# medical-genomics-group/hydra

Hardware: AMD Instinct MI355X
Metric: Gibbs markers/sec/iter (higher is better)
Workload: dtype f64

## Files before the change

### hydra_amd/capi.py

```python
import ctypes as C
import os
import numpy as np

_HERE = os.path.dirname(os.path.abspath(__file__))
LIB_PATH = os.path.join(_HERE, "libhgibbs.so")

ABI_SYMBOLS = [
    "hgibbs_last_error", "hgibbs_version", "hgibbs_create", "hgibbs_destroy", "hgibbs_comm_unique_id",
    "hgibbs_comm_init", "hgibbs_comm_init_external", "hgibbs_p2p_export", "hgibbs_p2p_import", "hgibbs_load_bed", "hgibbs_synth_bed", "hgibbs_dims", "hgibbs_get_bed",
    "hgibbs_marker_stats", "hgibbs_set_residual", "hgibbs_get_residual", "hgibbs_reduce_eps", "hgibbs_add_scalar",
    "hgibbs_update_marker", "hgibbs_dot_marker", "hgibbs_set_covariates", "hgibbs_cov_dot", "hgibbs_cov_update",
    "hydra_chain_set_covariates", "hydra_chain_gamma", "hgibbs_set_components", "hydra_chain_restore",
    "hydra_rng_to_boost_words", "hydra_rng_from_boost_words", "hydra_rng_shuffle", "hgibbs_set_model", "hgibbs_set_beta", "hgibbs_get_beta",
    "hgibbs_beta_sqnorm", "hgibbs_sweep", "hgibbs_set_option", "hgibbs_last_sweep_stats", "hgibbs_stream_ceiling", "hgibbs_debug_times", "hgibbs_resident_trace", "hydra_chain_create",
    "hydra_chain_destroy", "hydra_chain_iterate", "hydra_chain_state", "hydra_chain_csv_line", "hydra_chain_order",
    "hydra_chain_last_nnz", "hgibbs_score", "hgibbs_last_score_ms", "hgibbs_ld", "hgibbs_last_ld_ms",
    "hgibbs_ld_scores", "hgibbs_last_ld_scores_ms",
    "hgibbs_ld_mask", "hgibbs_last_ld_mask_ms", "hgibbs_ld_greedy", "hgibbs_ld_clump",
    "hgibbs_marker_dots", "hgibbs_last_marker_dots_ms", "hgibbs_marker_class_sums", "hgibbs_last_marker_class_sums_ms", "hgibbs_logit_null",
    "hgibbs_spa_roots", "hgibbs_last_spa_ms", "hgibbs_spa_pvalue",
    "hgibbs_king", "hgibbs_king_pairs", "hgibbs_king_pairs_get", "hgibbs_last_king_ms",
    "hgibbs_pca", "hgibbs_last_pca_ms", "hgibbs_region_var", "hgibbs_last_region_var_ms",
    "hgibbs_grm", "hgibbs_grm_info", "hgibbs_last_grm_ms",
    "hgibbs_grm_rowsums", "hgibbs_last_grm_rowsums_ms", "hgibbs_he_fit",
    "hgibbs_row_sums", "hgibbs_last_row_sums_ms", "hgibbs_hwe_exact",
    "hgibbs_sparse_begin", "hgibbs_sparse_put", "hgibbs_sparse_end", "hgibbs_sparse_counts", "hgibbs_sparse_get", "hgibbs_last_sparse_ms",
    "hgibbs_grand_seed", "hgibbs_grand_next", "hgibbs_ars_sample", "hgibbs_w_init", "hgibbs_w_marker_stats", "hgibbs_w_set_model",
    "hgibbs_w_reduce", "hgibbs_w_refresh_vi", "hgibbs_w_get_vi", "hgibbs_w_marker_sums", "hgibbs_w_sweep", "hgibbs_w_last_sweep_stats", "hgibbs_w_ars_device_probe",
    "hgibbs_w_get_beta", "hgibbs_w_set_beta", "hydraw_chain_create", "hydraw_chain_destroy", "hydraw_chain_set_covariates",
    "hydraw_chain_reseed_ars", "hydraw_chain_iterate", "hydraw_chain_state", "hydraw_chain_gamma", "hydraw_chain_order",
    "hydraw_chain_last_nnz", "hydraw_chain_csv_line", "hydraw_chain_restore",
]


class RngState(C.Structure):
    _fields_ = [("x", C.c_uint32 * 624), ("idx", C.c_uint32)]


class SweepStats(C.Structure):
    _fields_ = [("launches", C.c_uint64), ("nnz_updates", C.c_uint64), ("device_ms", C.c_double),
                ("kernel_ms_avg", C.c_double), ("carried_columns", C.c_uint64), ("working_launches", C.c_uint64),
                ("accepted_markers", C.c_uint64), ("streamed_columns", C.c_uint64), ("tiles_per_workgroup_min", C.c_uint32),
                ("tiles_per_workgroup_max", C.c_uint32), ("engine", C.c_uint32), ("walker", C.c_uint32), ("eps_sum_drift", C.c_double),
                ("rounds", C.c_uint64), ("events", C.c_uint64), ("advances", C.c_uint64), ("chunks", C.c_uint64), ("refolds", C.c_uint64), ("pivots", C.c_uint64), ("predicted", C.c_uint64), ("shader_mhz", C.c_double),
                ("ticks", C.c_uint64 * 16), ("refill", C.c_uint32), ("reserved_", C.c_uint32)]


class PcaReport(C.Structure):
    _fields_ = [("iters_run", C.c_int32), ("m_used", C.c_uint32), ("ritz_change", C.c_double), ("resid", C.c_double * 32)]


class SpaRoot(C.Structure):
    _fields_ = [("t", C.c_double * 2), ("K", C.c_double * 2), ("K2", C.c_double * 2), ("k2_0", C.c_double), ("s_lo", C.c_double),
                ("s_hi", C.c_double), ("iters", C.c_int32 * 2), ("flags", C.c_uint32), ("reserved_", C.c_uint32)]


class HeForm(C.Structure):
    _fields_ = [(k, C.c_double) for k in ("intercept", "slope", "h2", "intercept_se", "slope_se", "h2_se", "intercept_se_jk", "slope_se_jk",
                                         "h2_se_jk", "intercept_p", "slope_p", "intercept_p_jk", "slope_p_jk")]

# ... 91 lines not shown
    L.hgibbs_cov_dot.argtypes = [vp, C.c_int, C.c_double, dp]
    L.hgibbs_cov_update.argtypes = [vp, C.c_int, C.c_double]
    L.hydra_chain_set_covariates.argtypes = [vp, dp, C.c_int]
    L.hydra_chain_gamma.argtypes = [vp, dp, ip]
    L.hgibbs_set_components.argtypes = [vp, ip]
    L.hydra_chain_restore.argtypes = [vp, C.POINTER(RestartState)]
    L.hydra_rng_to_boost_words.argtypes = [C.POINTER(RngState), u32p]
    L.hydra_rng_from_boost_words.argtypes = [u32p, C.POINTER(RngState)]
    L.hydra_rng_shuffle.argtypes = [C.POINTER(RngState), ip, C.c_uint32]
    L.hgibbs_set_model.argtypes = [vp, C.c_int, C.c_int, ip, dp, dp]
    L.hgibbs_set_beta.argtypes = [vp, dp]
    L.hgibbs_get_beta.argtypes = [vp, dp, ip, dp]
    L.hgibbs_beta_sqnorm.argtypes = [vp, dp]
    L.hgibbs_sweep.argtypes = [vp, ip, C.c_double, dp, dp, u8p, C.POINTER(RngState), ip, u64p]
    L.hgibbs_set_option.argtypes = [vp, C.c_char_p, C.c_int64]
    L.hgibbs_last_sweep_stats.argtypes = [vp, C.POINTER(SweepStats)]
    L.hgibbs_stream_ceiling.argtypes = [vp, C.c_uint64, C.c_int, dp]
    L.hgibbs_debug_times.argtypes = [vp, C.POINTER(C.c_uint64)]
    L.hgibbs_resident_trace.argtypes = [vp, C.POINTER(C.c_uint64), C.c_uint64]
    L.hydra_chain_create.argtypes = [vp, C.POINTER(ModelDesc), dp, C.POINTER(vp)]
    L.hydra_chain_destroy.argtypes = [vp]
    L.hydra_chain_iterate.argtypes = [vp]
    L.hydra_chain_state.argtypes = [vp, dp, dp, dp, dp, ip, ip, C.POINTER(RngState)]
    L.hydra_chain_csv_line.argtypes = [vp, C.c_uint32, C.c_char_p, C.c_size_t]
    L.hydra_chain_order.argtypes = [vp]
    L.hydra_chain_order.restype = ip
    L.hydra_chain_last_nnz.argtypes = [vp]
    gp = C.POINTER(GrandState)
    L.hgibbs_grand_seed.argtypes = [gp, C.c_uint32]
    L.hgibbs_grand_seed.restype = None
# ... 636 lines not shown
        return cass, nnz.value

    def resident_trace(self):
        out = np.zeros((10, 4096), dtype=np.uint64)
        check(self.L.hgibbs_resident_trace(self.h, out.ctypes.data_as(C.POINTER(C.c_uint64)), out.size))
        return out

    def sweep_stats(self):
        s = SweepStats()
        check(self.L.hgibbs_last_sweep_stats(self.h, C.byref(s)))
        return {"launches": s.launches, "nnz_updates": s.nnz_updates, "device_ms": s.device_ms,
                "kernel_ms_avg": s.kernel_ms_avg, "carried_columns": s.carried_columns, "working_launches": s.working_launches,
                "accepted_markers": s.accepted_markers, "streamed_columns": s.streamed_columns,
                "tiles_per_workgroup_min": s.tiles_per_workgroup_min, "tiles_per_workgroup_max": s.tiles_per_workgroup_max,
                "engine": s.engine, "walker": s.walker, "refill": s.refill, "eps_sum_drift": s.eps_sum_drift, "rounds": s.rounds, "events": s.events,
                "advances": s.advances, "chunks": s.chunks, "refolds": s.refolds, "pivots": s.pivots, "predicted": s.predicted, "shader_mhz": s.shader_mhz, "ticks": list(s.ticks)}


class Chain:

    def __init__(self, dev, y, mS=None, groups=None, seed=1222, shuffle=1):
        self.dev = dev
        self.L = dev.L
        if mS is None:
            mS = np.array([[0.0, 0.0001, 0.001, 0.01]])
        self.mS = np.ascontiguousarray(mS, dtype=np.float64)
        self.G, self.K = self.mS.shape
        self.groups = None if groups is None else np.ascontiguousarray(groups, dtype=np.int32)
        y = np.ascontiguousarray(y, dtype=np.float64)
        assert y.shape[0] == dev.n_global
        d = ModelDesc(seed, shuffle, self.G, self.K, _ip(self.groups) if self.groups is not None else None, _dp(self.mS))
# ... 222 lines not shown
```

### hydra_amd/csrc/hg_resident.hip.h

```cpp
#pragma once

#include "hg_sweep.hip.h"

namespace hg {

constexpr int RS_WAVES = 8;
constexpr int RS_BLOCK = RS_WAVES * WAVE;
constexpr int RS_BMAX = 256;
constexpr int RS_NSH = 8;
constexpr int RS_RSH = 8;
constexpr int RS_GROW = 1024;
constexpr int RS_CROW = 1024;
constexpr int RS_RB = 2 * RS_BMAX;
constexpr int RS_MSG = 16;
constexpr int RS_PMAX = 4;
constexpr int RS_PFIRE = 16;
constexpr int RS_NB = 256;
constexpr int RS_TRACE = 4096;
constexpr int RS_TMAX = 2;
constexpr uint32_t RS_ONE = 1u << 24;
constexpr uint32_t RS_LOW = RS_ONE - 1u;
constexpr unsigned long long RS_ONE64 = 1ull << 56;
constexpr int RS_GFX = 32;
constexpr int RS_FG = 4, RS_FN = 256;
// ... 11 lines not shown
    uint32_t x = seq * 0x9E3779B1u ^ lo ^ (hi * 0x85EBCA77u);
    x ^= x >> 16;
    return x & 0xffffu;
}
constexpr unsigned long long RS_RONE = 1ull << 56;
__host__ __device__ inline unsigned long long rs_raw_value(unsigned long long d) { return (unsigned long long)((long long)(d << 8) >> 8); }
__host__ __device__ inline uint32_t rs_raw_count(unsigned long long d) { return (uint32_t)((d - rs_raw_value(d)) >> 56) & 0xffu; }
__host__ __device__ inline uint32_t rs_window_end(uint32_t C, uint32_t B, uint32_t M, uint32_t mask)
{
    const uint32_t e = (C + B) & ~mask;
    return e < M ? e : M;
}
__host__ __device__ inline uint32_t rs_msg_word0(uint32_t kf, uint32_t ncons, uint32_t seq, uint32_t lo, uint32_t hi) { return (kf << 28) | (rs_msg_check(seq, lo, hi) << 12) | ncons; }

struct ResState {
    uint32_t cursor, rng_idx, error, pad;
    unsigned long long rounds, events, advances, nnz, chunks, refolds, pivots, predicted;
    unsigned long long shader_ticks, wall_ticks;
    unsigned long long t[16];
};

struct ResParams {
    const uint8_t* bed;
    uint64_t stride;
    double* eps;
    uint32_t n_pad, n_local, M;
    double n_minus_1, n_total, eps_sum;
    const int32_t* order;
    const double* s_mave;
    const double* s_mstd;
    const double* s_bold;
// ... 18 lines not shown
    unsigned long long* racc;
    uint32_t* rcnt;
    unsigned long long* racc2;
    unsigned long long* gacc64;
    const unsigned long long* counts;
    unsigned long long* pacc;
    ResMsg* msg;
    ResState* state;
    double fx_scale, fx_unscale;
    unsigned long long timeout;
    unsigned long long* progress;
    unsigned long long rdv_timeout;
    unsigned long long* trace;
    int dbg;
    int pivots;
    int unused_;
    int early_advance;
    uint32_t wend_mask;
    int announce;
    int walker;
    const uint32_t* pred;
    int all_ada;
    int nranks, rank;
    unsigned char* mbox[RX_MAXR];
    unsigned long long sweep_id;
};

constexpr uint32_t RX_RING = 1024;
constexpr size_t RX_GBOX = 0;
constexpr size_t RX_RBOX = RX_GBOX + (size_t)RX_MAXR * 2 * RS_BMAX * 16;
constexpr size_t RX_HBOX = RX_RBOX + (size_t)RX_MAXR * RX_RING * 32;
// ... 1865 lines not shown
```

### hydra_amd/csrc/hg_walker2.hip.h

```cpp
#pragma once

namespace hg {

constexpr int W2_NBLK = 4;
constexpr uint32_t W2_RING = W2_NBLK * MT_N;
constexpr uint32_t W2_RR = 1024;
constexpr uint32_t W2_EV = 64;
constexpr uint32_t W2_PRED = 1024;
constexpr uint32_t W2_NB = 256;
constexpr int W2_NCH = 4;
constexpr uint32_t W2_NREC = 8;

enum {
    S_FPUB = 0,
    S_MPUB,
    S_CPUB,
    S_SEQPUB,
    S_RECSEQ,
    S_BLK,
    S_GPOS,
    S_PLD,
    S_PCUR,
    S_RDONE,
    S_EVN,
// ... 13 lines not shown
    R_FD,
    R_SEQ,
    R_PIN,
    R_PIQ,
    R_NEV,
    R_GPOSR,
    R_PFN,
    R_DB = 12,
    R_MQ = 14,
    R_SQ = 16,
    R_GSQ = 18,
    R_NMQ = 20,
    R_WORDS = 32
};
enum { RT_EXTEND = 0, RT_ADVANCE = 1, RT_PIVOT = 2, RT_EVENT = 3, RT_END = 4 };
enum { W2_ST_ROUNDS = 0, W2_ST_EVENTS, W2_ST_ADV, W2_ST_NNZ, W2_ST_CHUNKS, W2_ST_REFOLD, W2_ST_PIVOTS, W2_ST_PRED, W2_ST_ANN };

#define W2_ARRAYS(X)                                                                                                                          \
    X(double, tq, (size_t)W2_RING)         \
    X(double, zig_nx, 130)                                                                                                                    \
    X(double, zig_ny, 130)                                                                                                                    \
    X(double, htab, (size_t)4 * HT_LDS)                                                                                                       \
    X(double, qtab, (size_t)2 * HT_LDS)                                                                                                       \
    X(double, ftab, (size_t)RS_FG * (RS_FN + 1))                                                                                              \
    X(double, fscale, RS_FG)                                                                                                                  \
    X(double, mave, MR)                                                                               \
    X(double, mstd, MR)                                                                                                                       \
    X(double, bold, MR)                                                                                                                       \
    X(double, gsum, MR)                                                                                                     \
    X(double, nmis, MR)                                                                                                                       \
    X(double, dpr, Bz)                                                                               \
// ... 89 lines not shown
__device__ __forceinline__ Walk2Lds walk2_lds(uint32_t B)
{
    Walk2Lds sh;
    const Walk2Off off = walk2_offsets(B);
    uint32_t lb = (uint32_t)__builtin_amdgcn_readfirstlane((int)(uint32_t)(uintptr_t)(W2_LDS unsigned char*)hg_smem);
    asm volatile("" : "+s"(lb));
    W2_LDS unsigned char* const lbase = (W2_LDS unsigned char*)(uintptr_t)lb;
#define W2_X(type, name, count) sh.name = (W2_LDS type*)(lbase + off.name);
    W2_ARRAYS(W2_X)
#undef W2_X
    return sh;
}

#define W2_BEXPR pr.B
#define W2_PIVEXPR (pr.pivots != 0)
#define W2_PROLOGUE \
    const int tid = threadIdx.x, lane = tid & 63; \
    const int wave = __builtin_amdgcn_readfirstlane(tid >> 6); \
    const uint32_t B = W2_BEXPR, bmask = B - 1u, M = pr.M; \
    const uint32_t MR = 2u * B, mrmask = MR - 1u; \
    const int K = pr.K, GK = pr.GK; \
    const uint32_t W = pr.W, nsh = pr.nsh, rsh = pr.rsh; \
    const double n_total = pr.n_total, n_minus_1 = pr.n_minus_1, i_2sigE = pr.i_2sigE, eps_sum = pr.eps_sum, fx_unscale = pr.fx_unscale; \
    const unsigned long long timeout = pr.timeout; \
    const bool pivots = W2_PIVEXPR; \
    const uint32_t early_advance = (uint32_t)pr.early_advance; \
    const bool announce = pr.announce != 0 && !pivots; \
    const uint32_t rng_idx0 = pr.rng_idx; \
    ResMsg* const msg = pr.msg; \
    ResState* const state = pr.state; \
    unsigned long long* const trace = pr.trace; \
    unsigned long long* const progress = pr.progress; \
    const uint32_t* const gpred = pr.pred; \
    const double* const zig_ex = pr.zig.ex; \
    const double* const zig_ey = pr.zig.ey; \
    const Walk2Lds sh = walk2_lds(B); \
// ... 9 lines not shown
        const int ga = pr.s_ga[j]; \
        const int mk = pr.order[j]; \
        sh.marker[ms] = mk; \
        sh.ga[ms] = ga; \
        sh.bold[ms] = pr.s_bold[j]; \
        sh.mave[ms] = pr.s_mave[j]; \
        sh.mstd[ms] = pr.s_mstd[j]; \
        if constexpr (MISS) { \
            const unsigned long long* cn = pr.counts + 3ull * (unsigned long long)mk; \
            sh.gsum[ms] = (double)(cn[0] + 2ull * cn[1]); \
            sh.nmis[ms] = (double)cn[2]; \
        } \
    }; \
    auto tq_of = [&](uint32_t word) { \
        const double prob = (double)mt_temper(word) * (1.0 / 4294967296.0); \
        return log(1.0 / prob - 1.0) - 1e-9; \
    }; \
    auto aborted = [&]() { return w2_ld(sh.sw + S_ABORT) != 0u; }; \
    auto ended = [&]() { return w2_ld(sh.sw + S_END) != 0u; };

template <int DBG, int MISS, int BC, int RANKS, int DECIDE, int PIV>
__device__ __attribute__((noinline)) void w2_chain(const ResParams& prg)
{
    typedef const __attribute__((address_space(4))) ResParams w2_cparams;
    const unsigned long long pga = (unsigned long long)(uintptr_t)&prg;
    const unsigned long long pgu = ((unsigned long long)(uint32_t)__builtin_amdgcn_readfirstlane((int)(uint32_t)(pga >> 32)) << 32) |
                                   (uint32_t)__builtin_amdgcn_readfirstlane((int)(uint32_t)pga);
    w2_cparams& pr = *(w2_cparams*)(uintptr_t)pgu;
#undef W2_BEXPR
#define W2_BEXPR (BC ? (uint32_t)BC : pr.B)
#undef W2_PIVEXPR
#define W2_PIVEXPR (PIV != 0)
    W2_PROLOGUE
#undef W2_BEXPR
#define W2_BEXPR pr.B
#undef W2_PIVEXPR
#define W2_PIVEXPR (pr.pivots != 0)
    __builtin_amdgcn_s_setprio(3);
    constexpr bool decider = DECIDE != 0;
    const uint32_t nch = B >= 64u ? B / 64u : 1u;
    const uint32_t slot = (uint32_t)wave * 64u + (uint32_t)lane;
    const bool son = slot < B;
    const uint32_t sl = son ? slot : 0u;
    double dpr = 0.0, dp = 0.0, mave = 0.0, mstd = 0.0, boldn = 0.0, fsc = 0.0, gsm = 0.0, nms = 0.0;
    uint32_t fof = 0, sbt = 0, spi = 0;
    bool prd = false;
    uint32_t C = 0, Sx = 0, Fs = 0, base = 0, gposr = rng_idx0 % W2_RING;
    uint32_t gpa32[RS_NSH], gpb32[RS_NSH];
    unsigned long long gpa64[RS_NSH], gpb64[RS_NSH];
#pragma unroll
    for (int r = 0; r < RS_NSH; ++r) {
        gpa32[r] = gpb32[r] = 0u;
        gpa64[r] = gpb64[r] = 0ull;
    }
    typedef const __attribute__((address_space(1))) uint32_t* w2_g32;
    typedef const __attribute__((address_space(1))) unsigned long long* w2_g64;
    const w2_g32 gacc = (w2_g32)pr.gacc;
    const w2_g64 gacc64 = (w2_g64)pr.gacc64;
    uint32_t rno = 0;

    uint32_t seq = 0, nev = 0, pi = 0, evn = 0, pf_n = 0, gpos = rng_idx0, blk = 1u;
    uint32_t rdone_seen = 0, wpub_seen = 0, evw_seen = 0, pld_seen = W2_PRED, fpub_seen = 0, mpub_seen = m0;
    unsigned long long cm[W2_NCH] = {0ull, 0ull, 0ull, 0ull};
    uint32_t stat = 0;
    auto count = [&](uint32_t bits) { stat += (bits >> (uint32_t)lane) & 1u; };
    uint32_t err = 0;
    bool failed = false;
    unsigned long long tacc[8] = {0ull, 0ull, 0ull, 0ull, 0ull, 0ull, 0ull, 0ull};
    unsigned long long tmark = DBG ? wall_clock64() : 0ull;
    auto lap = [&](int i) {
        if (DBG && decider) {
            const unsigned long long now = wall_clock64();
            tacc[i] += now - tmark;
            tmark = now;
        }
    };
    auto pos_of_slot = [&](uint32_t s, uint32_t c) { return c + ((s - c) & bmask); };
    uint32_t nspin = 0;
// ... 263 lines not shown
            const int kx = inside ? (int)x : 0;
            uint32_t r = gposr + ((j - C) & bmask);
            r = r >= W2_RING ? r - W2_RING : r;
            const double f0 = sh.ftab[fof + (uint32_t)kx], f1 = sh.ftab[fof + (uint32_t)kx + 1u], tqv = sh.tq[r];
            const double fup = f0 + (x - (double)kx) * (f1 - f0);
            mymask = __ballot(act && (prd || !(inside && fup <= tqv)));
        }
        base = Fs;
        if (!decider) {
            if (lane == 0) *(W2_LDS u4_t*)(sh.ans + 4 * wave) = rs_u4((uint32_t)mymask, (uint32_t)(mymask >> 32), rno + 1u, 0u);
            ++rno;
            continue;
        }
        ++rno;
        lap(5);
        if (r_type != (uint32_t)RT_EXTEND) cm[0] = cm[1] = cm[2] = cm[3] = 0ull;
        cm[0] |= mymask;
        if (nch > 1u) {
            const unsigned long long t0 = wall_clock64();
            for (;;) {
                const u4_t a1 = *(const volatile W2_LDS u4_t*)(sh.ans + 4), a2 = *(const volatile W2_LDS u4_t*)(sh.ans + 8), a3 = *(const volatile W2_LDS u4_t*)(sh.ans + 12);
                const bool ok = w2_uni(a1.z) == rno && (nch < 3u || (w2_uni(a2.z) == rno && w2_uni(a3.z) == rno));
                if (ok) {
                    cm[1] |= ((unsigned long long)w2_uni(a1.y) << 32) | w2_uni(a1.x);
                    if (nch >= 3u) {
                        cm[2] |= ((unsigned long long)w2_uni(a2.y) << 32) | w2_uni(a2.x);
                        cm[3] |= ((unsigned long long)w2_uni(a3.y) << 32) | w2_uni(a3.x);
                    }
                    break;
                }
                if (spin_fail(t0)) {
                    failed = true;
                    break;
                }
            }
        }
        if (failed) break;
        lap(1);
        const uint32_t fc_rdone = __hip_atomic_load(sh.sw + S_RDONE, __ATOMIC_RELAXED, __HIP_MEMORY_SCOPE_WORKGROUP),
                       fc_wpub = __hip_atomic_load(sh.sw + S_WPUB, __ATOMIC_RELAXED, __HIP_MEMORY_SCOPE_WORKGROUP),
                       fc_evw = __hip_atomic_load(sh.sw + S_EVW, __ATOMIC_RELAXED, __HIP_MEMORY_SCOPE_WORKGROUP);
        if (lane == W2_ST_CHUNKS && (DBG || (stat & 255u) == 0u)) w2_gst(progress, ((unsigned long long)(uint32_t)__builtin_amdgcn_readlane((int)stat, W2_ST_ROUNDS) << 8) | 1u);
        if (PIV && pf_n) {
            if (Fs >= Sx) pf_n = 0;
            else {
                const uint32_t bF = w2_uni(sh.batch[Fs & bmask]);
                uint32_t drop = 0;
                while (drop < pf_n && w2_uni(sh.pf_msg[drop]) <= bF) ++drop;
                if (drop) {
                    if (lane == 0)
                        for (uint32_t f = drop; f < pf_n; ++f) {
                            sh.pf_pos[f - drop] = sh.pf_pos[f];
// ... 3 lines not shown
                            sh.pf_val[3 * (f - drop) + 1] = sh.pf_val[3 * f + 1];
                            sh.pf_val[3 * (f - drop) + 2] = sh.pf_val[3 * f + 2];
                        }
                    pf_n -= drop;
                    w2_lds_done();
                }
            }
        }
        if (gpos + B + 96u > blk * (uint32_t)MT_N && !wait_seen(blk, S_BLK, (gpos + B + 96u + (uint32_t)MT_N - 1u) / (uint32_t)MT_N)) break;
        count(1u << W2_ST_CHUNKS);
        bool found = false, announced = false;
        uint32_t qpos = 0, q_consumed = 0;
        int q_k = 0;
        double q_bnew = 0.0, q_bold = 0.0, q_mq = 0.0, q_sq = 0.0, q_gsq = 0.0, q_nmq = 0.0;
        {
            const uint32_t s0 = C & bmask, i0 = s0 >> 6, l0 = s0 & 63u;
            const unsigned long long lowm = (1ull << l0) - 1ull;
            for (;;) {
                uint32_t qs = 0xffffffffu;
#pragma unroll
                for (int t = 0; t <= W2_NCH; ++t) {
                    if ((uint32_t)t <= nch && qs == 0xffffffffu) {
                        uint32_t i = i0 + (uint32_t)t;
                        i = i >= nch ? i - nch : i;
                        unsigned long long mm = i == 0u ? cm[0] : (i == 1u ? cm[1] : (i == 2u ? cm[2] : cm[3]));
                        if (t == 0) mm &= ~lowm;
                        if ((uint32_t)t == nch) mm &= lowm;
                        if (mm) qs = i * 64u + (uint32_t)(__ffsll((long long)mm) - 1);
                    }
                }
                qs = w2_uni(qs);
                if (qs == 0xffffffffu) break;
                const uint32_t qc = pos_of_slot(qs, C);
                const uint32_t qi = qs >> 6, ql = qs & 63u;
                const uint32_t ms = qc & mrmask;
                uint32_t upos = gposr + (qc - C);
                upos = upos >= W2_RING ? upos - W2_RING : upos;
                const double bold_v = sh.bold[ms], num = sh.rnum[qc & (W2_RR - 1u)];
                const double cmq_v = sh.mave[ms], csq_v = sh.mstd[ms], cgsq_v = MISS ? sh.gsum[ms] : 0.0, cnmq_v = MISS ? sh.nmis[ms] : 0.0;
                const int ga_v = sh.ga[ms];
                const uint32_t word_v = sh.mt[upos];
                const uint32_t zp1 = upos + 1u == W2_RING ? 0u : upos + 1u, zp2 = zp1 + 1u == W2_RING ? 0u : zp1 + 1u;
                const uint32_t zw1 = sh.mt[zp1], zw2 = sh.mt[zp2];
                const double bold = w2_uni(bold_v);
                if (announce && !announced && bold != 0.0 && qc + 1u < Sx && (seq + 6u <= (uint32_t)RS_MSG || rdone_seen >= seq + 6u - (uint32_t)RS_MSG)) {
                    if (lane == 0) rs_store16(msg + ((seq + 1u) % RS_MSG), rs_u4(rs_msg_word0((uint32_t)RS_ANNOUNCE, qc - C + 1u, seq + 1u, 0u, 0u), seq + 1u, 0u, 0u));
                    announced = true;
                }
                const uint32_t zleft = blk * (uint32_t)MT_N - (gpos + (qc - C) + 1u);
// ... 18 lines not shown
                    const int lk = lane < K ? lane : 0;
                    const double den = sh.htab[g0 + lk], lpi = sh.htab[HT_LDS + g0 + lk], hlg = sh.htab[2 * HT_LDS + g0 + lk];
                    sdl = sh.htab[3 * HT_LDS + g0 + lk];
                    mk = num / (lk ? den : 1.0);
                    Lm = lk ? lpi - hlg + mk * num * i_2sigE : lpi;
                }
                const int kk = lane >> 3, l = lane & 7;
                const double Ll = __shfl(Lm, l, 64), Lk = __shfl(Lm, kk, 64);
                const bool on = kk < K - 1 && l < K;
                const double d = on ? Ll - Lk : 0.0;
                const double ex = exp(d);
                const bool bigp = on && l >= (kk ? kk : 1) && fabs(d) > 700.0;
                const unsigned long long bm = __ballot(bigp);
                double sum = ex, cur = ex;
#pragma unroll
                for (int x = 1; x < 8; ++x) {
                    cur = rs_dpp_f64<0x101>(cur);
                    if (x < K) sum += cur;
                }
                const bool anyb = ((bm >> (lane & ~7)) & 0xffull) != 0ull;
                const double thr = anyb ? 0.0 : 1.0 / sum;
                int k = K - 1;
                double acum = 0.0;
                bool fnd = false;
#pragma unroll
                for (int sidx = 0; sidx < 7; ++sidx) {
                    if (sidx + 1 < K) {
                        const double t = rs_readlane(thr, 8 * sidx);
                        acum = sidx ? acum + t : t;
                        if (!fnd && prob <= acum) {
                            k = sidx;
                            fnd = true;
                        }
                    }
                }
                k = w2_uni(k);
                double bnew = 0.0;
                uint32_t consumed = 0u, gerr = 0u;
                if (k > 0) {
                    const double mean_k = rs_readlane(mk, k), sd_k = rs_readlane(sdl, k);
                    if (zfast) {
                        bnew = z * sd_k + mean_k;
                        consumed = 2u;
                    } else {
                        if (lane == 0) {
                            RingGen g{sh.mt, zp1, zleft, 0u, 0u};
                            const ZigLds zt{sh.zig_nx, sh.zig_ny, zig_ex, zig_ey};
// ... 12 lines not shown
                    break;
                }
                if (k != 0 || bold != 0.0) {
                    found = true;
                    q_mq = w2_uni(cmq_v);
                    q_sq = w2_uni(csq_v);
                    q_gsq = w2_uni(cgsq_v);
                    q_nmq = w2_uni(cnmq_v);
                    qpos = qc;
                    q_k = k;
                    q_bnew = bnew;
                    q_bold = bold;
                    q_consumed = consumed;
                    break;
                }
                const unsigned long long bit = 1ull << ql;
                if (qi == 0u) cm[0] &= ~bit;
                else if (qi == 1u) cm[1] &= ~bit;
                else if (qi == 2u) cm[2] &= ~bit;
                else cm[3] &= ~bit;
            }
        }
        lap(3);
        if (failed) break;
        const uint32_t early_thr = early_advance;
        const bool early = !found && Fs < Sx && early_thr != 0u && Fs - C >= early_thr;
        if (!found && Fs < Sx && !early) {
            count(1u << W2_ST_REFOLD);
            if (!wait_seen(fpub_seen, S_FPUB, Fs + 1u)) break;
            lap(0);
            publish(RT_EXTEND, 0u, C, Sx, Sx, fpub_seen < Sx ? fpub_seen : Sx, 0u, 0.0, 0.0, 0.0, 0.0, 0.0);
            continue;
        }
        const uint32_t ncons = found ? qpos - C + 1u : (early ? Fs - C : Sx - C);
        const uint32_t Cn = C + ncons;
// ... 95 lines not shown
        publish(RT_END, 0u, C, Sx, Sx, 0u, 0u, 0.0, 0.0, 0.0, 0.0, 0.0);
        if (lane == 0) {
            w2_st(sh.sw + S_GPOS, gpos);
            w2_lds_done();
            w2_st(sh.sw + S_END, 1u);
            state->cursor = C;
            auto st = [&](int i) { return (uint32_t)__builtin_amdgcn_readlane((int)stat, i); };
            state->rounds = st(W2_ST_ROUNDS);
            state->events = st(W2_ST_EVENTS);
            state->advances = st(W2_ST_ADV);
            state->nnz = st(W2_ST_NNZ);
            state->chunks = st(W2_ST_CHUNKS);
            state->refolds = st(W2_ST_REFOLD);
            state->pivots = st(W2_ST_PIVOTS) + st(W2_ST_ANN);
            state->predicted = st(W2_ST_PRED);
            if (DBG)
                for (int i = 0; i < 8; ++i) state->t[i] = tacc[i];
        }
    }
}

template <int MISS, int RANKS>
__device__ __attribute__((noinline)) void w2_folder(const ResParams& pr)
{
    W2_PROLOGUE
    uint32_t Ff = 0, done = 0, fb = 0;
    unsigned long long t_idle = wall_clock64();
    auto poll_done = [&]() {
        uint32_t b = 0xffffffffu;
        if ((uint32_t)lane < rsh) b = __hip_atomic_load(pr.rcnt + (size_t)lane * RS_CROW, HG_RLX_AGENT) / cntR[(uint32_t)lane < W % rsh ? 0 : 1];
#pragma unroll
        for (int off = 32; off >= 1; off >>= 1) {
            const uint32_t o = (uint32_t)__shfl_xor((int)b, off, 64);
            b = o < b ? o : b;
// ... 329 lines not shown
        uint32_t np = 0;
        for (int ip = 0; ip < RS_PMAX; ++ip) np += (pivots && sh.pred[ip] < Sx0) ? 1u : 0u;
        sh.bl_pi[0] = 0u;
        sh.bl_np[0] = np;
        sh.bl_p0[0] = np ? sh.pred[0] : 0xffffffffu;
    }
    __syncthreads();

    if (wave < W2_NCH) {
        if ((uint32_t)wave < (B >= 64u ? B / 64u : 1u)) {
            if (wave == 0) {
                if (pr.nranks > 1) w2_chain<DBG, MISS, 0, 1, 1, 0>(pr);
                else if (!MISS && pr.pivots) {
                    if (B == 256u) w2_chain<DBG, MISS, 256, 0, 1, 1>(pr);
                    else w2_chain<DBG, MISS, 0, 0, 1, 1>(pr);
                } else if (B == 256u) w2_chain<DBG, MISS, 256, 0, 1, 0>(pr);
                else w2_chain<DBG, MISS, 0, 0, 1, 0>(pr);
            } else {
                if (pr.nranks > 1) w2_chain<DBG, MISS, 0, 1, 0, 0>(pr);
                else if (!MISS && pr.pivots) {
                    if (B == 256u) w2_chain<DBG, MISS, 256, 0, 0, 1>(pr);
                    else w2_chain<DBG, MISS, 0, 0, 0, 1>(pr);
                } else if (B == 256u) w2_chain<DBG, MISS, 256, 0, 0, 0>(pr);
                else w2_chain<DBG, MISS, 0, 0, 0, 0>(pr);
            }
        }
    } else if (wave == 4) {
        if (pr.nranks > 1) w2_folder<MISS, 1>(pr);
        else w2_folder<MISS, 0>(pr);
    }
    else if (wave == 5) w2_housekeeper<MISS>(pr);
    __syncthreads();
// ... 21 lines not shown
```

### hydra_amd/csrc/hgibbs.hip

```cpp
#include <hip/hip_runtime.h>
#include <rccl/rccl.h>

#include <algorithm>
#include <atomic>
#include <chrono>
#include <thread>
#include <cmath>
#include <cstdarg>
#include <cstdio>
#include <cstdlib>
#include <cstring>
#include <string>
#include <vector>

#include "../../include/hgibbs.h"
#include "hg_kernels.h"
#include "hg_sweep.hip.h"
#include "hg_resident.hip.h"

using namespace hg;

static thread_local std::string g_err;

static int fail(const char* fmt, ...)
// ... 117 lines not shown

    int engine = 0;
    bool res_all_ada = false;
    unsigned long long res_sweep_id = 0;
    bool engine_pinned = false;
    uint32_t window = 0;
    uint32_t res_cus = 0;
    int res_walker = 0;
    bool res_attr_set[20] = {};
    bool res_dead = false;
    uint32_t res_probed_w = 0;
    unsigned long long res_probe_id = 0;
    bool res_not_resident = false;
    int res_early = 24;
    int res_announce = 1;
    int res_wend = 1;
    int res_walker2_ranks = 1;
    double eps_abs_bound = 0.0;
    int res_refill = 0;
    int res_pivots = 0;
    unsigned char* res_acc = nullptr;
    ResMsg* res_msg = nullptr;
    ResState* res_state = nullptr;
    ResState* res_state_host = nullptr;
    ResParams* res_params = nullptr;
    ResParams* res_params_host = nullptr;
    unsigned long long* res_progress = nullptr;
    unsigned long long* res_progress_host = nullptr;
    hipStream_t aux_stream = nullptr;
    unsigned long long* res_trace = nullptr;
// ... 1121 lines not shown
        h->window = (uint32_t)value;
    } else if (!std::strcmp(name, "pivots")) {
        h->res_pivots = value != 0;
    } else if (!std::strcmp(name, "early_advance")) {
        if (value < 0 || value > 255) return fail("early_advance must be in [0,255]");
        h->res_early = (int)value;
    } else if (!std::strcmp(name, "refill")) {
        if (value < 0 || value > 2) return fail("refill must be 0 (auto), 1 (fused multiply-adds) or 2 (integer matrix products)");
        h->res_refill = (int)value;
    } else if (!std::strcmp(name, "walker2_ranks")) {
        h->res_walker2_ranks = value != 0;
    } else if (!std::strcmp(name, "window_end16")) {
        h->res_wend = value != 0;
    } else if (!std::strcmp(name, "announce")) {
        h->res_announce = value != 0;
    } else if (!std::strcmp(name, "walker")) {
        if (value < 0 || value > 2) return fail("walker must be 0 (auto), 1 (first) or 2 (second)");
        h->res_walker = (int)value;
    } else if (!std::strcmp(name, "res_cus")) {
        if (value < 0 || value > 4096) return fail("res_cus must be in [0,4096]");
        h->res_cus = (uint32_t)value;
    } else if (!std::strcmp(name, "res_deadline_ms")) {
        h->res_deadline_s = (double)value * 1e-3;
    } else if (!std::strcmp(name, "res_timeout_ms")) {
        if (value < 1) return fail("res_timeout_ms must be positive");
        h->res_timeout_s = (double)value * 1e-3;
    } else if (!std::strcmp(name, "p2p")) {
        h->p2p_enabled = value != 0;
    } else if (!std::strcmp(name, "force_split")) {
        h->force_split = value != 0;
    } else if (!std::strcmp(name, "w_kernel_timing")) {
        h->w_kernel_timing = value != 0;
    } else if (!std::strcmp(name, "debug_timing")) {
        h->debug_timing = value != 0;
    } else if (!std::strcmp(name, "sparse_piece")) {
        if (value < 0) return fail("sparse_piece must be >= 0 bytes (0 = automatic)");
        h->sparse_piece = (long long)value;
    } else if (!std::strcmp(name, "chunk")) {
        h->chunk = (int)value;
    } else {
        return fail("hgibbs_set_option: unknown option '%s'", name);
    }
    return 0;
}

int hgibbs_debug_times(hgibbs_t h, uint64_t* out8)
{
    if (!h || !out8) return fail("null argument");
    HIP_TRY(hipSetDevice(h->device));
    HIP_TRY(hipMemcpy(out8, h->dbg, 48 * sizeof(unsigned long long), hipMemcpyDeviceToHost));
    HIP_TRY(hipMemset(h->dbg, 0, 48 * sizeof(unsigned long long)));
    return 0;
}

int hgibbs_resident_trace(hgibbs_t h, uint64_t* out, uint64_t words)
{
    if (!h || !out) return fail("null argument");
    HIP_TRY(hipSetDevice(h->device));
// ... 200 lines not shown
        p.fx_scale = std::ldexp(1.0, ex);
        p.fx_unscale = std::ldexp(1.0, -ex);
    }
    p.timeout = (unsigned long long)(h->res_timeout_s * 1e8);
    p.rdv_timeout = (unsigned long long)(std::min(h->res_timeout_s, 0.1) * 1e8);
    p.dbg = h->debug_timing ? 1 : 0;
    p.pivots = pl.pivots;
    p.nranks = h->nranks > 1 ? h->nranks : 1;
    p.rank = h->nranks > 1 ? h->rank : 0;
    for (int r = 0; r < RX_MAXR; ++r) p.mbox[r] = (h->nranks > 1 && r < h->nranks) ? (unsigned char*)h->peer_base[r] + MBOX_RES_OFF : nullptr;
    p.all_ada = h->res_all_ada ? 1 : 0;
    p.walker = pl.walker;
    p.pred = h->pred;
    p.early_advance = p.nranks > 1 ? 0 : h->res_early;
    p.announce = h->res_announce;
    p.wend_mask = pl.wend_mask;
    {
        const uint32_t nchunk = (h->M + PRED_CHUNK - 1) / PRED_CHUNK;
        k_pred_count<<<nchunk, 256, 0, h->stream>>>(h->s_bold, h->M, h->pred_cnt);
        k_pred_scan<<<1, 1024, 0, h->stream>>>(h->pred_cnt, nchunk);
        k_pred_scatter<<<nchunk, 256, 0, h->stream>>>(h->s_bold, h->M, h->pred_cnt, nchunk, h->pred, nullptr);
        HIP_TRY(hipGetLastError());
    }
    p.sweep_id = ++h->res_sweep_id;
    p.trace = h->res_trace;
    p.progress = h->res_progress;
    HIP_TRY(hipMemsetAsync(h->res_progress, 0, 16 * sizeof(unsigned long long), h->stream));

    HIP_TRY(hipMemsetAsync(h->res_acc, 0, RES_ACC_BYTES, h->stream));
    HIP_TRY(hipMemsetAsync(h->res_msg, 0, RS_MSG * sizeof(ResMsg), h->stream));
// ... 90 lines not shown
    s.working_launches = st.rounds;
    s.kernel_ms_avg = st.rounds ? ms / (double)st.rounds : 0.0;
    s.accepted_markers = st.cursor;
    s.streamed_columns = h->M;
    s.tiles_per_workgroup_min = s.tiles_per_workgroup_max = (uint32_t)pl.T;
    s.engine = 2;
    s.walker = (uint32_t)pl.walker;
    s.refill = (uint32_t)pl.refill;
    s.rounds = st.rounds;
    s.events = st.events;
    s.advances = st.advances;
    s.chunks = st.chunks;
    s.refolds = st.refolds;
    s.pivots = st.pivots;
    s.predicted = st.predicted;
    for (int i = 0; i < 16; ++i) s.ticks[i] = st.t[i];
    s.shader_mhz = st.wall_ticks ? 100.0 * (double)st.shader_ticks / (double)st.wall_ticks : 0.0;
    {
        double r1[2];
        if (reduce_eps_all(h, r1)) return 1;
        s.eps_sum_drift = std::fabs(r1[0] - r0[0]);
    }
    if (timing) {
        auto ms = [](auto a, auto b) { return std::chrono::duration<double, std::milli>(b - a).count(); };
        std::fprintf(stderr, "[hgibbs] resident sweep: launch preparation %.3f ms, kernel wait %.3f ms (device %.3f), results + drift %.3f\n", ms(t_0, t_launch), ms(t_launch, t_kernel),
                     (double)s.device_ms, ms(t_kernel, std::chrono::steady_clock::now()));
    }
    return 0;
}

// ... 320 lines not shown
```

### include/hgibbs.h

```cpp
#ifndef HGIBBS_H
#define HGIBBS_H

#include <stddef.h>
#include <stdint.h>

#ifdef __cplusplus
extern "C" {
#endif

typedef struct hgibbs_ctx* hgibbs_t;

typedef struct {
    uint32_t x[624];
    uint32_t idx;
} hgibbs_rng_state;

const char* hgibbs_last_error(void);
int hgibbs_version(void);

int hgibbs_create(int device_id, hgibbs_t* out);
int hgibbs_destroy(hgibbs_t h);

int hgibbs_comm_unique_id(void* id128);
int hgibbs_comm_init(hgibbs_t h, int nranks, int rank, const void* id128);
// ... 39 lines not shown
int hgibbs_cov_update(hgibbs_t h, int c, double dgamma);

int hgibbs_set_model(hgibbs_t h, int G, int K, const int32_t* groups_host, const double* cVa_host,
                     const double* cVaI_host);

int hgibbs_set_beta(hgibbs_t h, const double* beta_host);
int hgibbs_set_components(hgibbs_t h, const int32_t* components_host);
int hgibbs_get_beta(hgibbs_t h, double* beta_host, int32_t* components_host, double* acum_host);
int hgibbs_beta_sqnorm(hgibbs_t h, double* bsq_host );

int hgibbs_sweep(hgibbs_t h, const int32_t* order_host, double sigmaE, const double* sigmaG_host,
                 const double* estPi_host, const uint8_t* adaV_host, hgibbs_rng_state* rng, int32_t* cass_host,
                 uint64_t* nnz_updates);

int hgibbs_set_option(hgibbs_t h, const char* name, int64_t value);
typedef struct {
    uint64_t launches;
    uint64_t nnz_updates;
    double device_ms;
    double kernel_ms_avg;
    uint64_t carried_columns;
    uint64_t working_launches;
    uint64_t accepted_markers;
    uint64_t streamed_columns;
    uint32_t tiles_per_workgroup_min;
    uint32_t tiles_per_workgroup_max;
    uint32_t engine;
    uint32_t walker;
    double eps_sum_drift;
    uint64_t rounds, events, advances, chunks, refolds;
    uint64_t pivots;
    uint64_t predicted;
    double shader_mhz;
    uint64_t ticks[16];
    uint32_t refill;
    uint32_t reserved_;
} hgibbs_sweep_stats;
int hgibbs_last_sweep_stats(hgibbs_t h, hgibbs_sweep_stats* out);
int hgibbs_stream_ceiling(hgibbs_t h, uint64_t bytes, int reps, double* gbps);
int hgibbs_debug_times(hgibbs_t h, uint64_t* out48);
int hgibbs_resident_trace(hgibbs_t h, uint64_t* out, uint64_t words);

int hgibbs_score(hgibbs_t h, int S, const double* a, const double* o, double* out);
int hgibbs_last_score_ms(hgibbs_t h, double* ms);

int hgibbs_row_sums(hgibbs_t h, int T, const double* tab, double* out);
int hgibbs_last_row_sums_ms(hgibbs_t h, double* ms);

int hgibbs_hwe_exact(uint32_t n_het, uint32_t n_hom_a, uint32_t n_hom_b, double* p);

int hgibbs_region_var(hgibbs_t h, int S, const double* a, const double* o, uint32_t nsets, const uint64_t* off, const uint32_t* idx,
// ... 190 lines not shown
```

Baseline: 9.379 million.

## Specialize walker2 chain for K=4 and keep candidate masks in lane registers

```diff
diff --git a/hydra_amd/capi.py b/hydra_amd/capi.py
--- a/hydra_amd/capi.py
+++ b/hydra_amd/capi.py
@@ -12,7 +12,7 @@
     "hgibbs_update_marker", "hgibbs_dot_marker", "hgibbs_set_covariates", "hgibbs_cov_dot", "hgibbs_cov_update",
     "hydra_chain_set_covariates", "hydra_chain_gamma", "hgibbs_set_components", "hydra_chain_restore",
     "hydra_rng_to_boost_words", "hydra_rng_from_boost_words", "hydra_rng_shuffle", "hgibbs_set_model", "hgibbs_set_beta", "hgibbs_get_beta",
-    "hgibbs_beta_sqnorm", "hgibbs_sweep", "hgibbs_set_option", "hgibbs_last_sweep_stats", "hgibbs_stream_ceiling", "hgibbs_debug_times", "hgibbs_resident_trace", "hydra_chain_create",
+    "hgibbs_beta_sqnorm", "hgibbs_sweep", "hgibbs_set_option", "hgibbs_walker_search", "hgibbs_last_sweep_stats", "hgibbs_stream_ceiling", "hgibbs_debug_times", "hgibbs_resident_trace", "hydra_chain_create",
     "hydra_chain_destroy", "hydra_chain_iterate", "hydra_chain_state", "hydra_chain_csv_line", "hydra_chain_order",
     "hydra_chain_last_nnz", "hgibbs_score", "hgibbs_last_score_ms", "hgibbs_ld", "hgibbs_last_ld_ms",
     "hgibbs_ld_scores", "hgibbs_last_ld_scores_ms",
@@ -43,7 +43,7 @@
                 ("accepted_markers", C.c_uint64), ("streamed_columns", C.c_uint64), ("tiles_per_workgroup_min", C.c_uint32),
                 ("tiles_per_workgroup_max", C.c_uint32), ("engine", C.c_uint32), ("walker", C.c_uint32), ("eps_sum_drift", C.c_double),
                 ("rounds", C.c_uint64), ("events", C.c_uint64), ("advances", C.c_uint64), ("chunks", C.c_uint64), ("refolds", C.c_uint64), ("pivots", C.c_uint64), ("predicted", C.c_uint64), ("shader_mhz", C.c_double),
-                ("ticks", C.c_uint64 * 16), ("refill", C.c_uint32), ("reserved_", C.c_uint32)]
+                ("ticks", C.c_uint64 * 16), ("refill", C.c_uint32), ("turned_down", C.c_uint32)]
 
 
 class PcaReport(C.Structure):
@@ -165,6 +165,7 @@
     L.hgibbs_beta_sqnorm.argtypes = [vp, dp]
     L.hgibbs_sweep.argtypes = [vp, ip, C.c_double, dp, dp, u8p, C.POINTER(RngState), ip, u64p]
     L.hgibbs_set_option.argtypes = [vp, C.c_char_p, C.c_int64]
+    L.hgibbs_walker_search.argtypes = [u64p, C.c_uint32, C.c_uint32, u32p, C.c_uint32]
     L.hgibbs_last_sweep_stats.argtypes = [vp, C.POINTER(SweepStats)]
     L.hgibbs_stream_ceiling.argtypes = [vp, C.c_uint64, C.c_int, dp]
     L.hgibbs_debug_times.argtypes = [vp, C.POINTER(C.c_uint64)]
@@ -831,7 +832,7 @@
                 "accepted_markers": s.accepted_markers, "streamed_columns": s.streamed_columns,
                 "tiles_per_workgroup_min": s.tiles_per_workgroup_min, "tiles_per_workgroup_max": s.tiles_per_workgroup_max,
                 "engine": s.engine, "walker": s.walker, "refill": s.refill, "eps_sum_drift": s.eps_sum_drift, "rounds": s.rounds, "events": s.events,
-                "advances": s.advances, "chunks": s.chunks, "refolds": s.refolds, "pivots": s.pivots, "predicted": s.predicted, "shader_mhz": s.shader_mhz, "ticks": list(s.ticks)}
+                "advances": s.advances, "chunks": s.chunks, "refolds": s.refolds, "pivots": s.pivots, "predicted": s.predicted, "turned_down": s.turned_down, "shader_mhz": s.shader_mhz, "ticks": list(s.ticks)}
 
 
 class Chain:
diff --git a/hydra_amd/csrc/hg_resident.hip.h b/hydra_amd/csrc/hg_resident.hip.h
--- a/hydra_amd/csrc/hg_resident.hip.h
+++ b/hydra_amd/csrc/hg_resident.hip.h
@@ -49,7 +49,7 @@
 __host__ __device__ inline uint32_t rs_msg_word0(uint32_t kf, uint32_t ncons, uint32_t seq, uint32_t lo, uint32_t hi) { return (kf << 28) | (rs_msg_check(seq, lo, hi) << 12) | ncons; }
 
 struct ResState {
-    uint32_t cursor, rng_idx, error, pad;
+    uint32_t cursor, rng_idx, error, turned_down;
     unsigned long long rounds, events, advances, nnz, chunks, refolds, pivots, predicted;
     unsigned long long shader_ticks, wall_ticks;
     unsigned long long t[16];
@@ -98,7 +98,7 @@
     unsigned long long* trace;
     int dbg;
     int pivots;
-    int unused_;
+    int bound_slack;
     int early_advance;
     uint32_t wend_mask;
     int announce;
diff --git a/hydra_amd/csrc/hg_walker2.hip.h b/hydra_amd/csrc/hg_walker2.hip.h
--- a/hydra_amd/csrc/hg_walker2.hip.h
+++ b/hydra_amd/csrc/hg_walker2.hip.h
@@ -51,7 +51,7 @@
     R_WORDS = 32
 };
 enum { RT_EXTEND = 0, RT_ADVANCE = 1, RT_PIVOT = 2, RT_EVENT = 3, RT_END = 4 };
-enum { W2_ST_ROUNDS = 0, W2_ST_EVENTS, W2_ST_ADV, W2_ST_NNZ, W2_ST_CHUNKS, W2_ST_REFOLD, W2_ST_PIVOTS, W2_ST_PRED, W2_ST_ANN };
+enum { W2_ST_ROUNDS = 0, W2_ST_EVENTS, W2_ST_ADV, W2_ST_NNZ, W2_ST_CHUNKS, W2_ST_REFOLD, W2_ST_PIVOTS, W2_ST_PRED, W2_ST_ANN, W2_ST_TURNED };
 
 #define W2_ARRAYS(X)                                                                                                                          \
     X(double, tq, (size_t)W2_RING)         \
@@ -171,12 +171,14 @@
 
 #define W2_BEXPR pr.B
 #define W2_PIVEXPR (pr.pivots != 0)
+#define W2_KEXPR pr.K
 #define W2_PROLOGUE \
     const int tid = threadIdx.x, lane = tid & 63; \
     const int wave = __builtin_amdgcn_readfirstlane(tid >> 6); \
     const uint32_t B = W2_BEXPR, bmask = B - 1u, M = pr.M; \
     const uint32_t MR = 2u * B, mrmask = MR - 1u; \
-    const int K = pr.K, GK = pr.GK; \
+    const int K = W2_KEXPR, GK = pr.GK; \
+    const double bound_slack = (double)pr.bound_slack; \
     const uint32_t W = pr.W, nsh = pr.nsh, rsh = pr.rsh; \
     const double n_total = pr.n_total, n_minus_1 = pr.n_minus_1, i_2sigE = pr.i_2sigE, eps_sum = pr.eps_sum, fx_unscale = pr.fx_unscale; \
     const unsigned long long timeout = pr.timeout; \
@@ -216,13 +218,35 @@
     }; \
     auto tq_of = [&](uint32_t word) { \
         const double prob = (double)mt_temper(word) * (1.0 / 4294967296.0); \
-        return log(1.0 / prob - 1.0) - 1e-9; \
+        return log(1.0 / prob - 1.0) - 1e-9 - bound_slack;  \
     }; \
     auto aborted = [&]() { return w2_ld(sh.sw + S_ABORT) != 0u; }; \
     auto ended = [&]() { return w2_ld(sh.sw + S_END) != 0u; };
 
-template <int DBG, int MISS, int BC, int RANKS, int DECIDE, int PIV>
-__device__ __attribute__((noinline)) void w2_chain(const ResParams& prg)
+template <class Get>
+__host__ __device__ __forceinline__ uint32_t w2_first_candidate(uint32_t s0, uint32_t nch, Get&& get)
+{
+    const uint32_t i0 = s0 >> 6;
+    const unsigned long long lowm = (1ull << (s0 & 63u)) - 1ull;
+    const unsigned long long m0 = get(i0);
+    unsigned long long mm = m0 & ~lowm;
+    if (mm) return i0 * 64u + (uint32_t)__builtin_ctzll(mm);
+    uint32_t i = i0;
+    for (uint32_t t = 1; t < nch; ++t) {
+        i = i + 1u == nch ? 0u : i + 1u;
+        mm = get(i);
+        if (mm) return i * 64u + (uint32_t)__builtin_ctzll(mm);
+    }
+    mm = m0 & lowm;
+    return mm ? i0 * 64u + (uint32_t)__builtin_ctzll(mm) : 0xffffffffu;
+}
+__host__ __device__ __forceinline__ unsigned long long w2_without_candidate(unsigned long long m, uint32_t i, uint32_t qs)
+{
+    return i == (qs >> 6) ? m & ~(1ull << (qs & 63u)) : m;
+}
+
+template <int DBG, int MISS, int BC, int RANKS, int DECIDE, int PIV, int KC>
+__device__ __forceinline__ void w2_chain_body(const ResParams& prg)
 {
     typedef const __attribute__((address_space(4))) ResParams w2_cparams;
     const unsigned long long pga = (unsigned long long)(uintptr_t)&prg;
@@ -233,11 +257,15 @@
 #define W2_BEXPR (BC ? (uint32_t)BC : pr.B)
 #undef W2_PIVEXPR
 #define W2_PIVEXPR (PIV != 0)
+#undef W2_KEXPR
+#define W2_KEXPR (KC ? KC : pr.K)
     W2_PROLOGUE
 #undef W2_BEXPR
 #define W2_BEXPR pr.B
 #undef W2_PIVEXPR
 #define W2_PIVEXPR (pr.pivots != 0)
+#undef W2_KEXPR
+#define W2_KEXPR pr.K
     __builtin_amdgcn_s_setprio(3);
     constexpr bool decider = DECIDE != 0;
     const uint32_t nch = B >= 64u ? B / 64u : 1u;
@@ -263,7 +291,11 @@
 
     uint32_t seq = 0, nev = 0, pi = 0, evn = 0, pf_n = 0, gpos = rng_idx0, blk = 1u;
     uint32_t rdone_seen = 0, wpub_seen = 0, evw_seen = 0, pld_seen = W2_PRED, fpub_seen = 0, mpub_seen = m0;
-    unsigned long long cm[W2_NCH] = {0ull, 0ull, 0ull, 0ull};
+    uint32_t cml = 0, cmh = 0;
+    auto cm_of = [&](uint32_t i) {
+        return ((unsigned long long)(uint32_t)__builtin_amdgcn_readlane((int)cmh, (int)i) << 32) | (uint32_t)__builtin_amdgcn_readlane((int)cml, (int)i);
+    };
+    const uint32_t ans_i = (lane >= 1 && (uint32_t)lane < nch) ? (uint32_t)lane : 0u;
     uint32_t stat = 0;
     auto count = [&](uint32_t bits) { stat += (bits >> (uint32_t)lane) & 1u; };
     uint32_t err = 0;
@@ -557,28 +589,32 @@
         }
         ++rno;
         lap(5);
-        if (r_type != (uint32_t)RT_EXTEND) cm[0] = cm[1] = cm[2] = cm[3] = 0ull;
-        cm[0] |= mymask;
-        if (nch > 1u) {
-            const unsigned long long t0 = wall_clock64();
-            for (;;) {
-                const u4_t a1 = *(const volatile W2_LDS u4_t*)(sh.ans + 4), a2 = *(const volatile W2_LDS u4_t*)(sh.ans + 8), a3 = *(const volatile W2_LDS u4_t*)(sh.ans + 12);
-                const bool ok = w2_uni(a1.z) == rno && (nch < 3u || (w2_uni(a2.z) == rno && w2_uni(a3.z) == rno));
-                if (ok) {
-                    cm[1] |= ((unsigned long long)w2_uni(a1.y) << 32) | w2_uni(a1.x);
-                    if (nch >= 3u) {
-                        cm[2] |= ((unsigned long long)w2_uni(a2.y) << 32) | w2_uni(a2.x);
-                        cm[3] |= ((unsigned long long)w2_uni(a3.y) << 32) | w2_uni(a3.x);
+        {
+            uint32_t al = 0u, ah = 0u;
+            if (nch > 1u) {
+                const uint32_t want = ans_i ? rno : 0u;
+                unsigned long long t0 = 0ull;
+                for (bool first = true;; first = false) {
+                    const u4_t a = *(const volatile W2_LDS u4_t*)(sh.ans + 4u * ans_i);
+                    if (__ballot(a.z != want) == 0ull) {
+                        al = a.x;
+                        ah = a.y;
+                        break;
                     }
-                    break;
-                }
-                if (spin_fail(t0)) {
-                    failed = true;
-                    break;
-                }
-            }
-        }
-        if (failed) break;
+                    if (first) t0 = wall_clock64();
+                    else if (spin_fail(t0)) {
+                        failed = true;
+                        break;
+                    }
+                }
+            }
+            if (failed) break;
+            al = lane == 0 ? (uint32_t)mymask : al;
+            ah = lane == 0 ? (uint32_t)(mymask >> 32) : ah;
+            const uint32_t keep = r_type != (uint32_t)RT_EXTEND ? 0u : 0xffffffffu;
+            cml = (cml & keep) | al;
+            cmh = (cmh & keep) | ah;
+        }
         lap(1);
         const uint32_t fc_rdone = __hip_atomic_load(sh.sw + S_RDONE, __ATOMIC_RELAXED, __HIP_MEMORY_SCOPE_WORKGROUP),
                        fc_wpub = __hip_atomic_load(sh.sw + S_WPUB, __ATOMIC_RELAXED, __HIP_MEMORY_SCOPE_WORKGROUP),
@@ -612,25 +648,11 @@
         int q_k = 0;
         double q_bnew = 0.0, q_bold = 0.0, q_mq = 0.0, q_sq = 0.0, q_gsq = 0.0, q_nmq = 0.0;
         {
-            const uint32_t s0 = C & bmask, i0 = s0 >> 6, l0 = s0 & 63u;
-            const unsigned long long lowm = (1ull << l0) - 1ull;
+            const uint32_t s0 = C & bmask;
             for (;;) {
-                uint32_t qs = 0xffffffffu;
-#pragma unroll
-                for (int t = 0; t <= W2_NCH; ++t) {
-                    if ((uint32_t)t <= nch && qs == 0xffffffffu) {
-                        uint32_t i = i0 + (uint32_t)t;
-                        i = i >= nch ? i - nch : i;
-                        unsigned long long mm = i == 0u ? cm[0] : (i == 1u ? cm[1] : (i == 2u ? cm[2] : cm[3]));
-                        if (t == 0) mm &= ~lowm;
-                        if ((uint32_t)t == nch) mm &= lowm;
-                        if (mm) qs = i * 64u + (uint32_t)(__ffsll((long long)mm) - 1);
-                    }
-                }
-                qs = w2_uni(qs);
+                const uint32_t qs = w2_first_candidate(s0, nch, cm_of);
                 if (qs == 0xffffffffu) break;
                 const uint32_t qc = pos_of_slot(qs, C);
-                const uint32_t qi = qs >> 6, ql = qs & 63u;
                 const uint32_t ms = qc & mrmask;
                 uint32_t upos = gposr + (qc - C);
                 upos = upos >= W2_RING ? upos - W2_RING : upos;
@@ -679,23 +701,34 @@
                 const unsigned long long bm = __ballot(bigp);
                 double sum = ex, cur = ex;
 #pragma unroll
-                for (int x = 1; x < 8; ++x) {
+                for (int x = 1; x < (KC ? KC : 8); ++x) {
                     cur = rs_dpp_f64<0x101>(cur);
                     if (x < K) sum += cur;
                 }
                 const bool anyb = ((bm >> (lane & ~7)) & 0xffull) != 0ull;
                 const double thr = anyb ? 0.0 : 1.0 / sum;
                 int k = K - 1;
-                double acum = 0.0;
-                bool fnd = false;
-#pragma unroll
-                for (int sidx = 0; sidx < 7; ++sidx) {
-                    if (sidx + 1 < K) {
+                if constexpr (KC != 0) {
+                    double ac[KC > 1 ? KC - 1 : 1];
+#pragma unroll
+                    for (int sidx = 0; sidx + 1 < KC; ++sidx) {
                         const double t = rs_readlane(thr, 8 * sidx);
-                        acum = sidx ? acum + t : t;
-                        if (!fnd && prob <= acum) {
-                            k = sidx;
-                            fnd = true;
+                        ac[sidx] = sidx ? ac[sidx - 1] + t : t;
+                    }
+#pragma unroll
+                    for (int sidx = KC - 2; sidx >= 0; --sidx) k = prob <= ac[sidx] ? sidx : k;
+                } else {
+                    double acum = 0.0;
+                    bool fnd = false;
+#pragma unroll
+                    for (int sidx = 0; sidx < 7; ++sidx) {
+                        if (sidx + 1 < K) {
+                            const double t = rs_readlane(thr, 8 * sidx);
+                            acum = sidx ? acum + t : t;
+                            if (!fnd && prob <= acum) {
+                                k = sidx;
+                                fnd = true;
+                            }
                         }
                     }
                 }
@@ -738,11 +771,10 @@
                     q_consumed = consumed;
                     break;
                 }
-                const unsigned long long bit = 1ull << ql;
-                if (qi == 0u) cm[0] &= ~bit;
-                else if (qi == 1u) cm[1] &= ~bit;
-                else if (qi == 2u) cm[2] &= ~bit;
-                else cm[3] &= ~bit;
+                count(1u << W2_ST_TURNED);
+                const unsigned long long cmn = w2_without_candidate(((unsigned long long)cmh << 32) | cml, (uint32_t)lane, qs);
+                cml = (uint32_t)cmn;
+                cmh = (uint32_t)(cmn >> 32);
             }
         }
         lap(3);
@@ -868,10 +900,22 @@
             state->refolds = st(W2_ST_REFOLD);
             state->pivots = st(W2_ST_PIVOTS) + st(W2_ST_ANN);
             state->predicted = st(W2_ST_PRED);
+            state->turned_down = st(W2_ST_TURNED);
             if (DBG)
                 for (int i = 0; i < 8; ++i) state->t[i] = tacc[i];
         }
     }
+}
+
+template <int DBG, int MISS, int BC, int RANKS, int DECIDE, int PIV>
+__device__ __attribute__((noinline)) void w2_chain(const ResParams& prg)
+{
+    w2_chain_body<DBG, MISS, BC, RANKS, DECIDE, PIV, 0>(prg);
+}
+template <int DBG, int MISS>
+__device__ __attribute__((noinline)) void w2_chain_k4(const ResParams& prg)
+{
+    w2_chain_body<DBG, MISS, 256, 0, 1, 0, 4>(prg);
 }
 
 template <int MISS, int RANKS>
@@ -1231,8 +1275,10 @@
                 else if (!MISS && pr.pivots) {
                     if (B == 256u) w2_chain<DBG, MISS, 256, 0, 1, 1>(pr);
                     else w2_chain<DBG, MISS, 0, 0, 1, 1>(pr);
-                } else if (B == 256u) w2_chain<DBG, MISS, 256, 0, 1, 0>(pr);
-                else w2_chain<DBG, MISS, 0, 0, 1, 0>(pr);
+                } else if (B == 256u) {
+                    if (K == 4) w2_chain_k4<DBG, MISS>(pr);
+                    else w2_chain<DBG, MISS, 256, 0, 1, 0>(pr);
+                } else w2_chain<DBG, MISS, 0, 0, 1, 0>(pr);
             } else {
                 if (pr.nranks > 1) w2_chain<DBG, MISS, 0, 1, 0, 0>(pr);
                 else if (!MISS && pr.pivots) {
diff --git a/hydra_amd/csrc/hgibbs.hip b/hydra_amd/csrc/hgibbs.hip
--- a/hydra_amd/csrc/hgibbs.hip
+++ b/hydra_amd/csrc/hgibbs.hip
@@ -155,6 +155,7 @@
     bool res_not_resident = false;
     int res_early = 24;
     int res_announce = 1;
+    int res_bound_slack = 0;
     int res_wend = 1;
     int res_walker2_ranks = 1;
     double eps_abs_bound = 0.0;
@@ -1306,6 +1307,9 @@
         h->res_wend = value != 0;
     } else if (!std::strcmp(name, "announce")) {
         h->res_announce = value != 0;
+    } else if (!std::strcmp(name, "bound_slack")) {
+        if (value < 0 || value > 1000000) return fail("bound_slack must be in [0,1000000]");
+        h->res_bound_slack = (int)value;
     } else if (!std::strcmp(name, "walker")) {
         if (value < 0 || value > 2) return fail("walker must be 0 (auto), 1 (first) or 2 (second)");
         h->res_walker = (int)value;
@@ -1334,6 +1338,23 @@
         return fail("hgibbs_set_option: unknown option '%s'", name);
     }
     return 0;
+}
+
+int hgibbs_walker_search(const uint64_t* masks, uint32_t nch, uint32_t cursor_slot, uint32_t* slots, uint32_t cap)
+{
+    if (!masks || (!slots && cap)) return fail("hgibbs_walker_search: null argument"), -1;
+    if (nch < 1 || nch > (uint32_t)W2_NCH || cursor_slot >= nch * 64u) return fail("hgibbs_walker_search: 1 <= nch <= %d and cursor_slot < 64 nch", W2_NCH), -1;
+    unsigned long long cm[W2_NCH] = {0ull, 0ull, 0ull, 0ull};
+    for (uint32_t i = 0; i < nch; ++i) cm[i] = masks[i];
+    uint32_t n = 0;
+    for (;;) {
+        const uint32_t qs = w2_first_candidate(cursor_slot, nch, [&](uint32_t i) { return cm[i]; });
+        if (qs == 0xffffffffu) break;
+        if (n >= cap) return fail("hgibbs_walker_search: more than %u candidates", cap), -1;
+        slots[n++] = qs;
+        for (uint32_t i = 0; i < (uint32_t)W2_NCH; ++i) cm[i] = w2_without_candidate(cm[i], i, qs);
+    }
+    return (int)n;
 }
 
 int hgibbs_debug_times(hgibbs_t h, uint64_t* out8)
@@ -1564,6 +1585,7 @@
     p.pred = h->pred;
     p.early_advance = p.nranks > 1 ? 0 : h->res_early;
     p.announce = h->res_announce;
+    p.bound_slack = h->res_bound_slack;
     p.wend_mask = pl.wend_mask;
     {
         const uint32_t nchunk = (h->M + PRED_CHUNK - 1) / PRED_CHUNK;
@@ -1684,6 +1706,7 @@
     s.refolds = st.refolds;
     s.pivots = st.pivots;
     s.predicted = st.predicted;
+    s.turned_down = st.turned_down;
     for (int i = 0; i < 16; ++i) s.ticks[i] = st.t[i];
     s.shader_mhz = st.wall_ticks ? 100.0 * (double)st.shader_ticks / (double)st.wall_ticks : 0.0;
     {
diff --git a/include/hgibbs.h b/include/hgibbs.h
--- a/include/hgibbs.h
+++ b/include/hgibbs.h
@@ -77,6 +77,7 @@
                  uint64_t* nnz_updates);
 
 int hgibbs_set_option(hgibbs_t h, const char* name, int64_t value);
+int hgibbs_walker_search(const uint64_t* masks, uint32_t nch, uint32_t cursor_slot, uint32_t* slots, uint32_t cap);
 typedef struct {
     uint64_t launches;
     uint64_t nnz_updates;
@@ -97,7 +98,7 @@
     double shader_mhz;
     uint64_t ticks[16];
     uint32_t refill;
-    uint32_t reserved_;
+    uint32_t turned_down;
 } hgibbs_sweep_stats;
 int hgibbs_last_sweep_stats(hgibbs_t h, hgibbs_sweep_stats* out);
 int hgibbs_stream_ceiling(hgibbs_t h, uint64_t bytes, int reps, double* gbps);
```

New measurement: 9.645 million (median of 6 runs). 2.8% higher.
